# ShenhanQian/KGDet

Hardware: AMD Instinct MI355X
Metric: training images/sec (whole node) KGDet R50-FPN 800x1333 (higher is better)
Workload: dtype f32 (3 MFMA products per multiply on hi/lo-split operands -- fp16 parts forward, bf16 parts for gradients --, f32 accumulate); 1 GPU; KGDet R50-FPN train step, 2 img/GPU at 800x1333 (padded 800x1344), DeformConv fwd/bwd + focal/moment losses + grad-clip + Adam; no collective at dp1 (one rank: nothing to exchange); global_batch=2, parallelism=dp1

## Files before the change

### kgdet_amd/csrc/bn_act.hip

```cpp
#include "common.h"

namespace kgdet {

namespace {

__device__ __forceinline__ float wave_sum(float v) {
#pragma unroll
  for (int d = 32; d > 0; d >>= 1) v += __shfl_xor(v, d);
  return v;
}

struct ChannelAffine {
  float s, t, mean, invstd;
};

__device__ __forceinline__ ChannelAffine channel_affine(const float *gamma, const float *beta, const float *mean,
                                                        const float *var, float eps, int c) {
  ChannelAffine a;
  a.mean = mean[c];
  a.invstd = 1.0f / sqrtf(var[c] + eps);
  a.s = (gamma ? gamma[c] : 1.0f) * a.invstd;
  a.t = (beta ? beta[c] : 0.0f) - a.mean * a.s;
  return a;
}
// ... 95 lines not shown
__global__ __launch_bounds__(256) void relu_sum_bwd_kernel(const float *__restrict__ gz, const float *__restrict__ z,
                                                           float *__restrict__ g, float *__restrict__ partial, int C, int HW,
                                                           int per, int P) {
  __shared__ float red[4];
  const int plane = blockIdx.y, c = plane % C, n = plane / C;
  const long long base = (long long)plane * HW;
  const int lo = blockIdx.x * per, hi = min(HW, lo + per);
  float s1 = 0.f;
  {
    typedef float f32x4u __attribute__((ext_vector_type(4), aligned(4)));
    const int hi4 = lo + ((hi - lo) & ~3);
    for (int i = lo + threadIdx.x * 4; i < hi4; i += 1024) {
      f32x4u v = *reinterpret_cast<const f32x4u *>(gz + base + i);
      if (RELU) {
        const f32x4u zv = *reinterpret_cast<const f32x4u *>(z + base + i);
        v[0] = zv[0] > 0.f ? v[0] : 0.f; v[1] = zv[1] > 0.f ? v[1] : 0.f; v[2] = zv[2] > 0.f ? v[2] : 0.f; v[3] = zv[3] > 0.f ? v[3] : 0.f;
        *reinterpret_cast<f32x4u *>(g + base + i) = v;
      }
      s1 += (v[0] + v[1]) + (v[2] + v[3]);
    }
    for (int i = hi4 + threadIdx.x; i < hi; i += 256) {
      float v = gz[base + i];
      if (RELU) { v = z[base + i] > 0.f ? v : 0.f; g[base + i] = v; }
      s1 += v;
    }
  }
  s1 = wave_sum(s1);
  if ((threadIdx.x & 63) == 0) red[threadIdx.x >> 6] = s1;
  __syncthreads();
  if (threadIdx.x == 0) partial[(long long)c * P + n * gridDim.x + blockIdx.x] = (red[0] + red[1]) + (red[2] + red[3]);
}

__global__ __launch_bounds__(256) void bn_fold_finish_kernel(const float *__restrict__ partial, int P,
                                                             const float *__restrict__ w, float *__restrict__ G,
                                                             const float *__restrict__ s, const float *__restrict__ mean,
                                                             const float *__restrict__ var, float eps,
                                                             float *__restrict__ gbeta, float *__restrict__ ggamma, int CK) {
  __shared__ float red[2][4];
  const int o = blockIdx.x;
  float sb = 0.f;
  for (int k = threadIdx.x; k < P; k += 256) sb += partial[(long long)o * P + k];
  float dot = 0.f;
  const float so = s[o];
  const float *wr = w + (long long)o * CK;
  float *gr = G ? G + (long long)o * CK : nullptr;
  if (gr) {
    for (int k = threadIdx.x; k < CK; k += 256) {
      const float gv = gr[k];
      dot += wr[k] * gv;
      gr[k] = gv * so;
    }
  }
  sb = wave_sum(sb);
  dot = wave_sum(dot);
  if ((threadIdx.x & 63) == 0) { red[0][threadIdx.x >> 6] = sb; red[1][threadIdx.x >> 6] = dot; }
  __syncthreads();
  if (threadIdx.x == 0) {
    const float b = (red[0][0] + red[0][1]) + (red[0][2] + red[0][3]);
    const float d = (red[1][0] + red[1][1]) + (red[1][2] + red[1][3]);
    if (gbeta) gbeta[o] = b;
    if (ggamma) ggamma[o] = (d - mean[o] * b) / sqrtf(var[o] + eps);
  }
}

namespace {

int chunks_for(int64_t planes, int64_t HW) {
  int64_t want = (4096 + planes - 1) / planes;
  const int64_t most = (HW + 1023) / 1024;
  if (want > most) want = most;
  return want < 1 ? 1 : (int)want;
}

}

}

using namespace kgdet;

__global__ __launch_bounds__(256) void bn_relu_maxpool_kernel(const float *__restrict__ x, const float *__restrict__ gamma,
                                                              const float *__restrict__ beta,
                                                              const float *__restrict__ mean,
                                                              const float *__restrict__ var, float eps,
                                                              float *__restrict__ y, int C, int H, int W, int Ho, int Wo) {
  const int plane = blockIdx.y, c = plane % C;
  const ChannelAffine a = channel_affine(gamma, beta, mean, var, eps, c);
  const float *xp = x + (long long)plane * H * W;
  float *yp = y + (long long)plane * Ho * Wo;
  for (int o = blockIdx.x * 256 + threadIdx.x; o < Ho * Wo; o += gridDim.x * 256) {
    const int i = o / Wo, j = o - i * Wo;
    float m = 0.f;
#pragma unroll
    for (int dy = -1; dy <= 1; ++dy) {
      const int r = 2 * i + dy;
      if (r < 0 || r >= H) continue;
#pragma unroll
      for (int dx = -1; dx <= 1; ++dx) {
        const int q = 2 * j + dx;
        if (q < 0 || q >= W) continue;
        m = fmaxf(m, xp[(long long)r * W + q] * a.s + a.t);
      }
    }
    yp[o] = m;
  }
}

extern "C" int kgdet_bn_relu_maxpool(const float *x, const float *gamma, const float *beta, const float *mean,
                                     const float *var, float eps, float *y, int64_t N, int32_t C, int32_t H, int32_t W,
                                     void *stream) {
  KGDET_CHECK_SHAPE(N >= 0 && C > 0 && H > 0 && W > 0, "bad sizes");
  if (N == 0) return KGDET_OK;
  KGDET_CHECK_SHAPE(x && y && mean && var, "null pointer");
  KGDET_CHECK_SHAPE(N * C <= 65535, "N*C = %lld exceeds the grid limit", (long long)(N * C));
  const int Ho = (H - 1) / 2 + 1, Wo = (W - 1) / 2 + 1;
  int chunks = (Ho * Wo + 1023) / 1024;
  hipLaunchKernelGGL(bn_relu_maxpool_kernel, dim3(chunks, (unsigned)(N * C)), dim3(256), 0, (hipStream_t)stream, x, gamma,
                     beta, mean, var, eps, y, C, H, W, Ho, Wo);
  KGDET_CHECK_LAUNCH("bn_relu_maxpool");
  return KGDET_OK;
}

extern "C" int32_t kgdet_bn_act_partials(int64_t N, int32_t C, int64_t HW) {
  if (N <= 0 || C <= 0 || HW <= 0) return 0;
  return (int32_t)(N * chunks_for(N * C, HW));
}

extern "C" int kgdet_bn_act_forward(const float *x, const float *gamma, const float *beta, const float *mean,
                                    const float *var, float eps, const float *residual, float *y, int64_t N, int32_t C,
                                    int64_t HW, int32_t relu, void *stream) {
  KGDET_CHECK_SHAPE(N >= 0 && C > 0 && HW >= 0 && HW < (1LL << 31), "bad sizes");
  if (N * HW == 0) return KGDET_OK;
  KGDET_CHECK_SHAPE(x && y && mean && var, "null pointer");
  KGDET_CHECK_SHAPE(N * C <= 65535, "N*C = %lld exceeds the grid limit", (long long)(N * C));
  const int chunks = chunks_for(N * C, HW);
  const int per = (int)(((HW + chunks - 1) / chunks + 3) / 4 * 4);
  dim3 grid(chunks, (unsigned)(N * C));
#define LAUNCH(RES, RELU)                                                                                      \
  hipLaunchKernelGGL((bn_act_fwd_kernel<RES, RELU>), grid, dim3(256), 0, (hipStream_t)stream, x, gamma, beta, \
                     mean, var, eps, residual, y, C, (int)HW, per)
  if (residual) { if (relu) LAUNCH(true, true); else LAUNCH(true, false); }
  else { if (relu) LAUNCH(false, true); else LAUNCH(false, false); }
#undef LAUNCH
  KGDET_CHECK_LAUNCH("bn_act_forward");
  return KGDET_OK;
}

extern "C" int kgdet_bn_act_backward(const float *grad_y, const float *x, const float *y, const float *gamma,
                                     const float *beta, const float *mean, const float *var, float eps,
                                     int32_t has_residual, int32_t relu, float *grad_x, float *grad_residual,
                                     float *partial, float *sums, int64_t N, int32_t C, int64_t HW, void *stream) {
  KGDET_CHECK_SHAPE(N >= 0 && C > 0 && HW >= 0 && HW < (1LL << 31), "bad sizes");
  if (N * HW == 0) return KGDET_OK;
  KGDET_CHECK_SHAPE(grad_y && x && mean && var && partial, "null pointer");
  KGDET_CHECK_SHAPE(!(has_residual && relu) || (y && grad_residual),
                    "residual + relu needs the forward output and a grad_residual buffer");
  KGDET_CHECK_SHAPE(N * C <= 65535, "N*C = %lld exceeds the grid limit", (long long)(N * C));
  const int chunks = chunks_for(N * C, HW);
  const int per = (int)(((HW + chunks - 1) / chunks + 3) / 4 * 4);
  const int P = (int)(N * chunks);
  dim3 grid(chunks, (unsigned)(N * C));
#define LAUNCH(RES, RELU)                                                                                        \
  hipLaunchKernelGGL((bn_act_bwd_kernel<RES, RELU>), grid, dim3(256), 0, (hipStream_t)stream, grad_y, x, y, gamma, \
                     beta, mean, var, eps, grad_x, grad_residual, partial, C, (int)HW, per, P)
  if (has_residual) { if (relu) LAUNCH(true, true); else LAUNCH(true, false); }
  else { if (relu) LAUNCH(false, true); else LAUNCH(false, false); }
#undef LAUNCH
  KGDET_CHECK_LAUNCH("bn_act_backward");
  if (sums) {
    hipLaunchKernelGGL(bn_partial_sum, dim3((2 * C + 255) / 256), dim3(256), 0, (hipStream_t)stream, partial, sums, 2 * C,
                       P);
    KGDET_CHECK_LAUNCH("bn_partial_sum");
  }
  return KGDET_OK;
}

extern "C" int kgdet_bn_fold_backward(const float *grad_z, const float *z, int32_t relu, float *g, float *partial, int64_t N,
                                      int32_t C, int64_t HW, void *stream) {
  KGDET_CHECK_SHAPE(N >= 0 && C > 0 && HW >= 0 && HW < (1LL << 31), "bad sizes");
  if (N * HW == 0) return KGDET_OK;
  KGDET_CHECK_SHAPE(grad_z && partial && (!relu || (z && g)), "null pointer");
  KGDET_CHECK_SHAPE(N * C <= 65535, "N*C = %lld exceeds the grid limit", (long long)(N * C));
  const int chunks = chunks_for(N * C, HW);
  const int per = (int)(((HW + chunks - 1) / chunks + 3) / 4 * 4);
  const int P = (int)(N * chunks);
  dim3 grid(chunks, (unsigned)(N * C));
  if (relu)
    hipLaunchKernelGGL(relu_sum_bwd_kernel<true>, grid, dim3(256), 0, (hipStream_t)stream, grad_z, z, g, partial, C, (int)HW,
                       per, P);
  else
    hipLaunchKernelGGL(relu_sum_bwd_kernel<false>, grid, dim3(256), 0, (hipStream_t)stream, grad_z, z, g, partial, C,
                       (int)HW, per, P);
  KGDET_CHECK_LAUNCH("bn_fold_backward");
  return KGDET_OK;
}

extern "C" int kgdet_bn_fold_finish(const float *partial, int32_t P, const float *w, float *G, const float *s,
                                    const float *mean, const float *var, float eps, float *grad_beta, float *grad_gamma,
                                    int32_t O, int32_t CK, void *stream) {
  KGDET_CHECK_SHAPE(O > 0 && CK > 0 && P > 0, "bad sizes");
  KGDET_CHECK_SHAPE(partial && w && s && mean && var, "null pointer");
// ... 7 lines not shown
```

### kgdet_amd/csrc/dense_forward.hip

```cpp
#include "dense_common.h"

namespace kgdet {

__global__ __launch_bounds__(256) void conv1x1_pack(const float *__restrict__ w, int O, int C, int T, int transpose,
                                                    unsigned char *__restrict__ img, unsigned char *__restrict__ img_t,
                                                    int f16_forward) {
  if (gridDim.y == 2) {
    transpose = blockIdx.y;
    img = blockIdx.y ? img_t : img;
  }
  const bool f16 = f16_forward && !transpose;
  f16_saturate_on();
  const int M = transpose ? C : O, K = transpose ? O : C;
  const int k16s = (K + kTK - 1) / kTK;
  const long long total = (long long)((M + kTM - 1) / kTM) * k16s * T * 2 * kTM;
  for (long long i = blockIdx.x * 256LL + threadIdx.x; i < total; i += gridDim.x * 256LL) {
    const int row = (int)(i % kTM);
    const int khalf = (int)((i / kTM) & 1);
    const long long st = i / (2 * kTM);
    const int t = (int)(st % T);
    const int k16 = (int)((st / T) % k16s), mt = (int)(st / ((long long)T * k16s));
    const int m = mt * kTM + row, k0 = k16 * kTK + khalf * 8;
    float v[8];
#pragma unroll
    for (int j = 0; j < 8; ++j) {
      const long long o = transpose ? k0 + j : m, ch = transpose ? m : k0 + j;
      v[j] = (m < M && k0 + j < K) ? w[(o * C + ch) * T + (transpose ? T - 1 - t : t)] : 0.0f;
    }
    bf16x8 hi, lo;
    if (f16) {
#pragma unroll
      for (int j = 0; j < 8; ++j) v[j] *= kF16WeightScale;
      split8_t<true>(v, hi, lo);
    } else {
      split8(v, hi, lo);
    }
    unsigned char *dst = img + st * kStage + khalf * (kTM * 16) + row * 16;
    *reinterpret_cast<bf16x8 *>(dst) = hi;
    *reinterpret_cast<bf16x8 *>(dst + kPart) = lo;
  }
}

constexpr int kPackDescWords = 6;
__global__ __launch_bounds__(256) void conv1x1_pack_multi(const long long *__restrict__ desc, int n) {
  int lo = 0, hi = n - 1;
  while (lo < hi) {
    const int mid = (lo + hi + 1) >> 1;
    if ((int)(desc[mid * kPackDescWords + 4] & 0xffffffffLL) <= (int)blockIdx.x) lo = mid; else hi = mid - 1;
  }
  const long long *d = desc + lo * kPackDescWords;
  const float *w = reinterpret_cast<const float *>(d[0]);
  const float *scale = reinterpret_cast<const float *>(d[5]);
  const int O = (int)(d[3] >> 32), C = (int)(d[3] & 0xffffffffLL), T = (int)((d[4] >> 32) & 0xffff);
  const bool f16_forward = (d[4] >> 62) & 1;
  f16_saturate_on();
  const long long i = (long long)((int)blockIdx.x - (int)(d[4] & 0xffffffffLL)) * 256 + threadIdx.x;
#pragma unroll
  for (int transpose = 0; transpose < 2; ++transpose) {
    unsigned char *img = reinterpret_cast<unsigned char *>(d[1 + transpose]);
    const int M = transpose ? C : O, K = transpose ? O : C;
    const int k16s = (K + kTK - 1) / kTK;
    const long long total = (long long)((M + kTM - 1) / kTM) * k16s * T * 2 * kTM;
    if (!transpose && T == 9) {
      if (i >= total / 9) continue;
      const int row = (int)(i % kTM), khalf = (int)((i / kTM) & 1);
      const long long s2 = i / (2 * kTM);
      const int k16 = (int)(s2 % k16s), mt = (int)(s2 / k16s);
      const int m = mt * kTM + row, k0 = k16 * kTK + khalf * 8;
      float r[72];
      const f32x4 *src = reinterpret_cast<const f32x4 *>(w + ((long long)min(m, M - 1) * C + k0) * 9);
#pragma unroll
      for (int q = 0; q < 18; ++q) {
        const f32x4 u = src[q];
        r[4 * q] = u[0]; r[4 * q + 1] = u[1]; r[4 * q + 2] = u[2]; r[4 * q + 3] = u[3];
      }
      const float sc9 = (scale && m < M) ? scale[m] : 1.0f;
#pragma unroll
      for (int t = 0; t < 9; ++t) {
        float v[8];
#pragma unroll
        for (int j = 0; j < 8; ++j) v[j] = m < M ? r[j * 9 + t] * sc9 : 0.0f;
        bf16x8 hi8, lo8;
        if (f16_forward) {
#pragma unroll
          for (int j = 0; j < 8; ++j) v[j] *= kF16WeightScale;
          split8_t<true>(v, hi8, lo8);
        } else {
          split8(v, hi8, lo8);
        }
        unsigned char *dst = img + (s2 * 9 + t) * kStage + khalf * (kTM * 16) + row * 16;
        *reinterpret_cast<bf16x8 *>(dst) = hi8;
        *reinterpret_cast<bf16x8 *>(dst + kPart) = lo8;
      }
      continue;
    }
    if (i >= total) continue;
    const int row = (int)(i % kTM);
    const int khalf = (int)((i / kTM) & 1);
    const long long st = i / (2 * kTM);
    const int t = (int)(st % T);
    const int k16 = (int)((st / T) % k16s), mt = (int)(st / ((long long)T * k16s));
    const int m = mt * kTM + row, k0 = k16 * kTK + khalf * 8;
    float v[8];
#pragma unroll
    for (int j = 0; j < 8; ++j) {
      const long long o = transpose ? k0 + j : m, ch = transpose ? m : k0 + j;
      v[j] = (m < M && k0 + j < K) ? w[(o * C + ch) * T + (transpose ? T - 1 - t : t)] : 0.0f;
      if (scale && m < M && k0 + j < K) v[j] *= scale[o];
    }
    bf16x8 hi8, lo8;
    if (f16_forward && !transpose) {
#pragma unroll
      for (int j = 0; j < 8; ++j) v[j] *= kF16WeightScale;
      split8_t<true>(v, hi8, lo8);
    } else {
      split8(v, hi8, lo8);
    }
    unsigned char *dst = img + st * kStage + khalf * (kTM * 16) + row * 16;
    *reinterpret_cast<bf16x8 *>(dst) = hi8;
    *reinterpret_cast<bf16x8 *>(dst + kPart) = lo8;
  }
}

constexpr int kPF = 4;

template <int TAPS, int NW = 4, bool F16 = false>
__global__ __launch_bounds__(128 * NW) void conv_nn(const unsigned char *__restrict__ img,
                                                      const float *__restrict__ x, float *__restrict__ y, int M, int K,
                                                      int H, int W, int n_mt, int n_nt, int tiles, int ksplit,
                                                      long long part_stride, int Hin, int Win, int stride,
                                                      const float *__restrict__ bias,
                                                      const float *__restrict__ residual, int relu,
    const float *__restrict__ gate = nullptr) {
  constexpr int TN = 32 * NW, kPartB = 2 * TN * 16, kBuf = kStage + 2 * kPartB;
  __shared__ __attribute__((aligned(16))) unsigned char smem[2 * kBuf];
  if constexpr (F16) f16_saturate_on();
  const int unit = xcd_tile(blockIdx.x, tiles * ksplit);
  if (unit >= tiles * ksplit) return;
  const int part = unit % ksplit, tile = unit / ksplit;
  const int tid = threadIdx.x, lane = tid & 63, wave = tid >> 6, wm = wave & 1, wn = wave >> 1;
  const int n_local = tid % TN, kq = tid / TN;
  const int N = H * W;
  const int S = TAPS * ((K + kTK - 1) / kTK), per = (S + ksplit - 1) / ksplit;
  const int s_begin = part * per, s_end = max(s_begin, min(S, s_begin + per));
  const int stages = s_end - s_begin;
  struct Regs {
    f32x4 a;
    float v[4];
    unsigned live;
  };
  const int mt = tile % n_mt, nt = (tile / n_mt) % n_nt, b = tile / (n_mt * n_nt);
  const int n0 = nt * TN;
  const int p = min(n0 + n_local, N - 1);
  unsigned ok = 1u;
  if (TAPS == 9) {
    const int h = (p / W) * stride, w = (p - (p / W) * W) * stride;
    ok = 0u;
#pragma unroll
    for (int t = 0; t < 9; ++t) {
      const int hh = h + t / 3 - 1, ww = w + t % 3 - 1;
      ok |= (hh >= 0 && hh < Hin && ww >= 0 && ww < Win) ? (1u << t) : 0u;
    }
  }
  const int Nin = Hin * Win;
  const int pin = stride == 1 ? p : (p / W) * stride * Win + (p - (p / W) * W) * stride;
  const float *xb = x + (long long)b * K * Nin + pin;
  const unsigned char *ai = img + (long long)mt * S * kStage + (tid & 511) * 16;

  f32x16 acc[2];
#pragma unroll
  for (int i = 0; i < 2; ++i)
#pragma unroll
    for (int r = 0; r < 16; ++r) acc[i][r] = 0.0f;

  auto issue = [&](int s, Regs &R) {
    const int sc = s_begin + min(s, stages - 1);
    R.a = *reinterpret_cast<const f32x4 *>(ai + (long long)sc * kStage);
    const int c16 = sc / TAPS, t = sc - c16 * TAPS;
    int shift = 0;
    R.live = 1u;
    if (TAPS == 9) {
      R.live = (ok >> t) & 1u;
      shift = R.live ? (t / 3 - 1) * Win + (t % 3 - 1) : 0;
    }
    const float *xp = xb + (long long)(c16 * kTK + kq * 4) * Nin + shift;
    if (TAPS == 1 && (K & (kTK - 1)) && c16 == K / kTK) {
#pragma unroll
      for (int j = 0; j < 4; ++j) R.v[j] = xb[(long long)min(c16 * kTK + kq * 4 + j, K - 1) * Nin];
    } else {
#pragma unroll
      for (int j = 0; j < 4; ++j) R.v[j] = xp[(long long)j * Nin];
    }
  };
  auto commit = [&](int buf, const Regs &R) {
    unsigned char *As = smem + buf * kBuf, *Bs = As + kStage;
    *reinterpret_cast<f32x4 *>(As + (tid & 511) * 16) = R.a;
    uint2 hi, lo;
    split_pair_t<F16>(R.live ? R.v[0] : 0.0f, R.live ? R.v[1] : 0.0f, hi.x, lo.x);
    split_pair_t<F16>(R.live ? R.v[2] : 0.0f, R.live ? R.v[3] : 0.0f, hi.y, lo.y);
    unsigned char *dst = Bs + (kq >> 1) * (TN * 16) + n_local * 16 + (kq & 1) * 8;
    *reinterpret_cast<uint2 *>(dst) = hi;
    *reinterpret_cast<uint2 *>(dst + kPartB) = lo;
  };
  auto multiply = [&](int buf) {
// ... 529 lines not shown
    const long long u4 = (long long)n_mt * ((hw + 127) / 128) * B, u5 = (long long)n_mt * ((hw + 159) / 160) * B;
    const long long c4 = ((u4 + 255) / 256) * 4, c5 = ((u5 + 255) / 256) * 5;
    if (force_nw == 5 || (force_nw == 0 && u4 >= 200 && u5 >= 200 && c5 * 10 <= c4 * 9)) {
      p.NW = 5;
      p.n_nt = (int)((hw + 159) / 160);
    }
  }
  p.tiles = (long long)n_mt * p.n_nt * B;
  p.ks = nn_ksplit(p.tiles, taps * ((K + kTK - 1) / kTK));
  if (p.patch && p.tiles < 200) {
    const int chunks = K / kTK;
    double best = 1e30;
    p.ks = 1;
    for (int ks = 1; ks <= 8 && ks * 2 <= chunks; ++ks) {
      const double out_mb = (double)B * M * Ho * Wo * 4e-6;
      const double cost = (double)((p.tiles * ks + 255) / 256) * ((chunks + ks - 1) / ks) + 0.114 * out_mb * ks;
      if (cost < best) { best = cost; p.ks = ks; }
    }
  }
  static const int force_ks = env_int("KGDET_CONV_KS", 0);
  if (force_ks > 0) p.ks = force_ks;
  static const int force_halves = env_int("KGDET_CONV_HALVES", -1);
  p.halves = p.patch && p.NB == 4 &&
             (force_halves >= 0 ? force_halves != 0 : ((p.ks == 1 && p.tiles > 256 && p.tiles < 400) || M <= 64));
  return p;
}

enum NNCloser { kCloseStore = 0, kCloseSumEpilogue = 1, kCloseSumBiasAct = 2, kCloseSum = 3 };
NNCloser nn_closer(int ks, long long HW, bool epilogue) {
  if (ks <= 1) return kCloseStore;
  if (!epilogue) return kCloseSum;
  return HW % 2 == 0 ? kCloseSumEpilogue : kCloseSumBiasAct;
}

}

}

using namespace kgdet;

extern "C" size_t kgdet_conv_packed_bytes(int32_t M, int32_t K, int32_t taps) {
  if (M <= 0 || K <= 0 || (taps == 9 && K % kTK) || (taps != 1 && taps != 9)) return 0;
  return (size_t)pack_items(M, K, taps) * 32;
}

extern "C" int kgdet_conv_pack_fmt(const float *w, int32_t O, int32_t C, int32_t taps, int32_t transpose, void *packed,
                                   int32_t operand_format, void *stream) {
  const int M = transpose ? C : O, K = transpose ? O : C;
  KGDET_CHECK_SHAPE(taps == 1 || taps == 9, "taps must be 1 (1x1) or 9 (3x3)");
  KGDET_CHECK_SHAPE(O > 0 && C > 0 && (taps == 1 || K % kTK == 0), "reduction length %d is not a multiple of 16", K);
  KGDET_CHECK_SHAPE(w && packed, "null pointer");
  const long long blocks = (pack_items(M, K, taps) + 255) / 256;
  hipLaunchKernelGGL(conv1x1_pack, dim3((unsigned)(blocks > 65535 ? 65535 : blocks)), dim3(256), 0, (hipStream_t)stream, w,
                     O, C, taps, transpose, (unsigned char *)packed, (unsigned char *)nullptr, operand_format == 1 ? 1 : 0);
  KGDET_CHECK_LAUNCH("conv_pack");
  return KGDET_OK;
}

extern "C" int kgdet_conv_pack(const float *w, int32_t O, int32_t C, int32_t taps, int32_t transpose, void *packed,
                               void *stream) {
  return kgdet_conv_pack_fmt(w, O, C, taps, transpose, packed, 0, stream);
}

extern "C" int kgdet_conv_pack_both_fmt(const float *w, int32_t O, int32_t C, int32_t taps, void *packed, void *packed_t,
                                        int32_t forward_format, void *stream) {
  KGDET_CHECK_SHAPE(taps == 1 || taps == 9, "taps must be 1 (1x1) or 9 (3x3)");
  KGDET_CHECK_SHAPE(O > 0 && C > 0 && (taps == 1 || (O % kTK == 0 && C % kTK == 0)), "O and C must be multiples of 16");
  KGDET_CHECK_SHAPE(w && packed && packed_t, "null pointer");
  const long long blocks = pack_both_blocks(O, C, taps);
  hipLaunchKernelGGL(conv1x1_pack, dim3((unsigned)(blocks > 32768 ? 32768 : blocks), 2), dim3(256), 0,
                     (hipStream_t)stream, w, O, C, taps, 0, (unsigned char *)packed, (unsigned char *)packed_t,
                     forward_format == 1 ? 1 : 0);
  KGDET_CHECK_LAUNCH("conv_pack_both");
  return KGDET_OK;
}

extern "C" int kgdet_conv_pack_both(const float *w, int32_t O, int32_t C, int32_t taps, void *packed, void *packed_t,
                                    void *stream) {
  return kgdet_conv_pack_both_fmt(w, O, C, taps, packed, packed_t, 0, stream);
}

extern "C" int64_t kgdet_conv_pack_blocks(int32_t O, int32_t C, int32_t taps) {
  if (O <= 0 || C <= 0 || (taps == 9 && (O % kTK || C % kTK)) || (taps != 1 && taps != 9)) return 0;
  return pack_both_blocks(O, C, taps);
}

extern "C" int kgdet_conv_pack_multi(const int64_t *desc_dev, int32_t n, int64_t total_blocks, void *stream) {
  KGDET_CHECK_SHAPE(desc_dev && n > 0 && total_blocks > 0 && total_blocks < (1LL << 31), "bad descriptor table");
  hipLaunchKernelGGL(conv1x1_pack_multi, dim3((unsigned)total_blocks), dim3(256), 0, (hipStream_t)stream,
                     (const long long *)desc_dev, n);
  KGDET_CHECK_LAUNCH("conv_pack_multi");
  return KGDET_OK;
}

extern "C" size_t kgdet_conv_apply_workspace_bytes(int64_t B, int32_t M, int32_t K, int32_t H, int32_t W,
                                                    int32_t taps, int32_t stride) {
  if (B <= 0 || M <= 0 || K <= 0 || H <= 0 || W <= 0 || (taps == 9 && K % kTK) || stride < 1 || stride > 2) return 0;
  const long long HW = (long long)((H + stride - 1) / stride) * ((W + stride - 1) / stride);
  const int ks = plan_nn(B, M, K, H, W, taps, stride).ks;
  return ks > 1 ? (size_t)ks * B * M * HW * sizeof(float) : 0;
}

extern "C" int kgdet_conv_apply_plan(int64_t B, int32_t M, int32_t K, int32_t H, int32_t W, int32_t taps, int32_t stride,
                                     int32_t out[KGDET_CONV_APPLY_PLAN_WORDS]) {
  KGDET_CHECK_SHAPE(out, "null pointer");
  KGDET_CHECK_SHAPE(B > 0 && M > 0 && K > 0 && H > 0 && W > 0 && (long long)H * W < (1LL << 30), "bad sizes");
  KGDET_CHECK_SHAPE(taps == 1 || taps == 9, "taps must be 1 (1x1) or 9 (3x3)");
  KGDET_CHECK_SHAPE(stride == 1 || stride == 2, "stride must be 1 or 2");
  KGDET_CHECK_SHAPE(taps == 1 || K % kTK == 0, "reduction length %d is not a multiple of 16", K);
  const NNPlan p = plan_nn(B, M, K, H, W, taps, stride);
  KGDET_CHECK_SHAPE(p.tiles < (1LL << 28), "too many tiles");
  const long long HW = (long long)((H + stride - 1) / stride) * ((W + stride - 1) / stride);
  const int32_t words[KGDET_CONV_APPLY_PLAN_WORDS] = {
      p.patch, p.TX, p.TY, p.NB, p.NW, p.ks, p.halves, (int32_t)p.tiles, p.n_nt, nn_closer(p.ks, HW, true), nn_closer(p.ks, HW, false)};
  for (int i = 0; i < KGDET_CONV_APPLY_PLAN_WORDS; ++i) out[i] = words[i];
  return KGDET_OK;
}

extern "C" int kgdet_conv_apply_epilogue_fmt(const void *packed, const float *x, float *y, const float *bias,
                                             const float *residual, int32_t relu, int64_t B, int32_t M, int32_t K,
                                             int32_t H, int32_t W, int32_t taps, int32_t stride, int32_t operand_format,
                                             void *workspace, size_t workspace_bytes, void *stream) {
  return kgdet_conv_apply_gated_fmt(packed, x, y, bias, residual, relu, nullptr, B, M, K, H, W, taps, stride, operand_format,
                                    workspace, workspace_bytes, stream);
}

extern "C" int kgdet_conv_apply_gated_fmt(const void *packed, const float *x, float *y, const float *bias,
                                          const float *residual, int32_t relu, const float *gate, int64_t B, int32_t M,
                                          int32_t K, int32_t H, int32_t W, int32_t taps, int32_t stride,
                                          int32_t operand_format, void *workspace, size_t workspace_bytes, void *stream) {
  const bool f16 = operand_format == 1;
  KGDET_CHECK_SHAPE(B >= 0 && M > 0 && K > 0 && H >= 0 && W >= 0 && (long long)H * W < (1LL << 30), "bad sizes");
  KGDET_CHECK_SHAPE(taps == 1 || taps == 9, "taps must be 1 (1x1) or 9 (3x3)");
  KGDET_CHECK_SHAPE(stride == 1 || stride == 2, "stride must be 1 or 2");
  KGDET_CHECK_SHAPE(taps == 1 || K % kTK == 0, "reduction length %d is not a multiple of 16", K);
  const int Ho = (H + stride - 1) / stride, Wo = (W + stride - 1) / stride;
  const long long HW = (long long)Ho * Wo;
  if (B * HW == 0) return KGDET_OK;
  KGDET_CHECK_SHAPE(packed && x && y, "null pointer");
  const NNPlan plan = plan_nn(B, M, K, H, W, taps, stride);
  const int n_mt = (M + kTM - 1) / kTM, n_nt = plan.n_nt;
  const long long tiles = plan.tiles;
  KGDET_CHECK_SHAPE(tiles < (1LL << 28), "too many tiles");
  const int ks = plan.ks;
  const long long part_stride = B * M * HW;
  if (ks > 1) {
    KGDET_CHECK_SHAPE(workspace && workspace_bytes >= (size_t)ks * part_stride * sizeof(float), "workspace too small");
    KGDET_CHECK_SHAPE(part_stride % 2 == 0, "B*M*Ho*Wo must be even");
    KGDET_CHECK_SHAPE(!gate || HW % 2 == 0, "a gated K-split convolution needs an even pixel count");
  }
  const unsigned grid = (unsigned)((tiles * ks + 7) / 8) * 8;
  float *dst = ks > 1 ? (float *)workspace : y;
  const float *k_bias = ks > 1 ? nullptr : bias, *k_residual = ks > 1 ? nullptr : residual, *k_gate = ks > 1 ? nullptr : gate;
  const int k_relu = ks > 1 ? 0 : relu;
  const unsigned char *img = (const unsigned char *)packed;
  if (plan.patch) {
    auto launch = [&](auto bf16_kernel, auto f16_kernel, unsigned g, unsigned threads) {
      launch_fmt(f16, bf16_kernel, f16_kernel, g, threads, stream, img, x, dst, M, K, H, W, n_mt, plan.tiles_x, n_nt, (int)tiles,
                 ks, part_stride, plan.TX, plan.TY, k_bias, k_residual, k_relu, k_gate);
    };
    if (plan.NB == 5)
      launch(conv3x3_patch4<4, 5, false>, conv3x3_patch4<4, 5, true>, grid, 256);
    else if (plan.halves)
      launch(conv3x3_patch4<2, 4, false>, conv3x3_patch4<2, 4, true>, (unsigned)((tiles * ks * 2 + 7) / 8) * 8, 128);
    else
      launch(conv3x3_patch4<4, 4, false>, conv3x3_patch4<4, 4, true>, grid, 256);
  } else {
// ... 88 lines not shown
```

### kgdet_amd/csrc/dense_grad_weight.hip

```cpp
#include "dense_common.h"

namespace kgdet {

struct ConvFoldArgs {
  const float *w, *s, *mean, *var, *bn_partial;
  float *grad_beta, *grad_gamma;
  float eps;
  int P;
};
template <bool T9>
__global__ __launch_bounds__(1024) void conv_wsum_fold(const float *__restrict__ parts, float *__restrict__ out, int C,
                                                       long long stride, int count, const ConvFoldArgs f) {
  extern __shared__ float row_s[];
  __shared__ float red[2][16];
  const int o = blockIdx.x, CK = T9 ? 9 * C : C;
  const int nthr = blockDim.x, tid = threadIdx.x;
  const float so = f.s[o];
  const float *wr = f.w + (long long)o * CK;
  const float *pr = parts + (long long)o * CK;
  float *gr = out + (long long)o * CK;
  float dot = 0.0f, sb = 0.0f;
  for (int q = tid; q < CK; q += nthr) {
    float g0 = 0.0f;
    int k = 0;
// ... 394 lines not shown
#pragma unroll
        for (int pt = 0; pt < 2; ++pt) {
#pragma unroll
          for (int i = 0; i < 2; ++i) fa[ks][pt][i] = *reinterpret_cast<const bf16x8 *>(A + ks * kPKS + pt * kPPart + i * 32 * 16);
#pragma unroll
          for (int i = 0; i < kPNI; ++i) fb[ks][pt][i] = *reinterpret_cast<const bf16x8 *>(Bp + ks * kPKS + pt * kPPart + i * 32 * 16);
        }
#pragma unroll
      for (int ks = 0; ks < 2; ++ks) {
#pragma unroll
        for (int mi = 0; mi < 2; ++mi)
#pragma unroll
          for (int ni = 0; ni < kPNI; ++ni)
            acc[mi][ni] = __builtin_amdgcn_mfma_f32_32x32x16_bf16(fa[ks][1][mi], fb[ks][0][ni], acc[mi][ni], 0, 0, 0);
#pragma unroll
        for (int mi = 0; mi < 2; ++mi)
#pragma unroll
          for (int ni = 0; ni < kPNI; ++ni)
            acc[mi][ni] = __builtin_amdgcn_mfma_f32_32x32x16_bf16(fa[ks][0][mi], fb[ks][1][ni], acc[mi][ni], 0, 0, 0);
#pragma unroll
        for (int mi = 0; mi < 2; ++mi)
#pragma unroll
          for (int ni = 0; ni < kPNI; ++ni)
            acc[mi][ni] = __builtin_amdgcn_mfma_f32_32x32x16_bf16(fa[ks][0][mi], fb[ks][0][ni], acc[mi][ni], 0, 0, 0);
      }
    };
    if (n > 0) {
      __syncthreads();
      for (int j = 0; j < n; j += 2) {
        multiply(0);
        __syncthreads();
        if (j + 1 < n) {
          multiply(1);
          __syncthreads();
        }
      }
    }
    float *out = partial + (long long)split * M * N;
#pragma unroll
    for (int mi = 0; mi < 2; ++mi)
#pragma unroll
      for (int ni = 0; ni < kPNI; ++ni) {
        const int nn = nt * kTN + wn * (32 * kPNI) + ni * 32 + (lane & 31);
#pragma unroll
        for (int r = 0; r < 16; ++r) {
          const int m = mt * kTM + wm * 64 + mi * 32 + (r & 3) + 8 * (r >> 2) + 4 * (lane >> 5);
          if (m < M && nn < N) out[(long long)m * N + nn] = acc[mi][ni][r];
        }
      }
  }
}

template <int TAPS, bool ALIGNED>
__global__ __launch_bounds__(kPThreads, 1) void conv_ntp(const float *__restrict__ a, const float *__restrict__ bm,
                                                         float *__restrict__ partial, int M, int N, int L, int B, int n_mt,
                                                         int n_nt, int stages_per_image, int per, int H, int W, int Cin,
                                                         int units, float *__restrict__ row_sums = nullptr, int rs_stride = 0) {
  extern __shared__ __attribute__((aligned(16))) unsigned char smem[];
  const int unit = units > 0 ? xcd_tile(blockIdx.x, units) : (int)blockIdx.x;
  if (units > 0 && unit >= units) return;
  if (threadIdx.x >= kPCons * 64)
    conv_ntp_role<TAPS, true, ALIGNED>(a, bm, partial, M, N, L, B, n_mt, n_nt, stages_per_image, per, H, W, Cin, unit, smem, row_sums, rs_stride);
  else
    conv_ntp_role<TAPS, false, ALIGNED>(a, bm, partial, M, N, L, B, n_mt, n_nt, stages_per_image, per, H, W, Cin, unit, smem, row_sums, rs_stride);
}

}


__global__ __launch_bounds__(256) void pad_rows2(const float *__restrict__ a, float *__restrict__ ap, long long rows_a,
                                                 const float *__restrict__ b, float *__restrict__ bp, long long rows_b, int W,
                                                 int Wp) {
  const float *src = blockIdx.y ? b : a;
  float *dst = blockIdx.y ? bp : ap;
  const long long n = (blockIdx.y ? rows_b : rows_a) * Wp;
  for (long long i = (long long)blockIdx.x * 256 + threadIdx.x; i < n; i += (long long)gridDim.x * 256) {
    const long long r = i / Wp;
    const int c = (int)(i - r * Wp);
    dst[i] = c < W ? src[r * W + c] : 0.0f;
  }
}

__global__ __launch_bounds__(256) void conv_s2_gather9(const float *__restrict__ x, float *__restrict__ col, int C, int H, int W,
                                                       int Ho, int Wo, long long rows) {
  const int HWo = Ho * Wo;
  const long long total = rows * HWo;
  for (long long i = (long long)blockIdx.x * 256 + threadIdx.x; i < total; i += (long long)gridDim.x * 256) {
    const long long r = i / HWo;
    const int p = (int)(i - r * HWo), oy = p / Wo, ox = p - oy * Wo;
    const long long b = r / C;
    const int c = (int)(r - b * C);
    const float *xp = x + r * (long long)H * W;
    float *cp = col + (b * 9 * C + c) * (long long)HWo + p;
#pragma unroll
    for (int t = 0; t < 9; ++t) {
      const int yy = 2 * oy + t / 3 - 1, xx = 2 * ox + t % 3 - 1;
      cp[(long long)t * C * HWo] = (yy >= 0 && yy < H && xx >= 0 && xx < W) ? xp[(long long)yy * W + xx] : 0.0f;
    }
  }
}

namespace kgdet {

namespace {

int nt_splits(int tiles, int total_stages) {
  const int most = (total_stages + 31) / 32;
  double best = 1e30;
  const int s_max = 2 * ((256 + tiles - 1) / tiles) < 128 ? 2 * ((256 + tiles - 1) / tiles) : 128;
  for (int s = 1; s <= s_max; ++s) {
    const double t = (double)((tiles * s + 255) / 256) / s;
    if (t < best) best = t;
  }
  int splits = 0;
  for (int s = 1; s <= s_max && !splits; ++s)
    if ((double)((tiles * s + 255) / 256) / s <= best * (1.0 + 1e-9) && tiles * s >= 224 && tiles * s <= 256) splits = s;
  for (int s = s_max; s >= 1 && !splits; --s)
    if ((double)((tiles * s + 255) / 256) / s <= best * (1.0 + 1e-9)) splits = s;
  if (splits > most) splits = most;
  if (splits > 128) splits = 128;
  return splits < 1 ? 1 : splits;
}

int fold_threads(int cols) {
  const int t = (cols + 63) / 64 * 64;
  return t < 64 ? 64 : (t > 1024 ? 1024 : t);
}

struct GWPlan {
  int n_mt, n_nt, tiles, splits;
  bool use_ntp, padded;
  long long W, Wp, L, Lp;
  int spi, per;
  size_t copies_at, rows_at, bytes;
};
GWPlan plan_gw(long long B, int O, int C, long long H, long long W, int taps) {
  GWPlan p;
  p.W = W;
  p.Wp = (W + 3) & ~3LL;
  p.L = H * W;
  p.Lp = H * p.Wp;
  p.n_mt = (O + kTM - 1) / kTM;
  p.n_nt = taps == 9 ? 9 * C / kTN : (C + kTN - 1) / kTN;
  p.tiles = p.n_mt * p.n_nt;
  p.splits = nt_splits(p.tiles, (int)(B * ((p.Lp + kTK - 1) / kTK)));
  const long long widest = O > C ? O : C;
  p.use_ntp = taps == 9 ? W >= 4 && p.L >= 4 && p.L <= (1LL << 21) && widest * p.Lp < (1LL << 30)
                        : W % 4 != 0 && W >= 4 && widest * p.L < (1LL << 30);
  p.padded = W % 4 != 0 && !p.use_ntp;
  const long long stage = p.use_ntp ? kPK : kTK, len = p.use_ntp ? p.L : p.Lp;
  p.spi = (int)((len + stage - 1) / stage);
  p.per = (int)((B * p.spi + p.splits - 1) / p.splits);
  p.bytes = (size_t)p.splits * O * C * taps * sizeof(float);
  p.copies_at = align_up(p.bytes, 256);
  if (p.Wp != W) p.bytes = p.copies_at + (size_t)B * (O + C) * p.Lp * sizeof(float);
  p.rows_at = align_up(p.bytes, 256);
  p.bytes = p.rows_at + (size_t)p.splits * O * sizeof(float);
  return p;
}

int launch_gw(const GWPlan &p, int taps, const float *grad_y, const float *x, float *grad_w, long long B, int O, int C, int H,
              void *workspace, void *stream, const ConvFoldArgs *fold, int wsum_C) {
  unsigned char *ws = static_cast<unsigned char *>(workspace);
  const hipStream_t st = (hipStream_t)stream;
  float *partials = reinterpret_cast<float *>(ws);
  float *row_sums = (fold && !fold->bn_partial) ? reinterpret_cast<float *>(ws + p.rows_at) : nullptr;
  if (p.padded) {
    float *gyp = reinterpret_cast<float *>(ws + p.copies_at), *xp = gyp + (size_t)B * O * p.Lp;
// ... 79 lines not shown

}

using namespace kgdet;

extern "C" size_t kgdet_conv1x1_grad_weight_workspace_bytes(int64_t B, int32_t O, int32_t C, int64_t HW) {
  if (B <= 0 || O <= 0 || C <= 0 || HW <= 0) return 0;
  return plan_gw(B, O, C, 1, HW, 1).bytes;
}

extern "C" size_t kgdet_conv3x3_grad_weight_workspace_bytes(int64_t B, int32_t O, int32_t C, int32_t H, int32_t W) {
  if (B <= 0 || O <= 0 || C <= 0 || H <= 0 || W <= 0) return 0;
  return plan_gw(B, O, C, H, W, 9).bytes;
}

extern "C" int kgdet_conv_grad_weight_plan(int64_t B, int32_t O, int32_t C, int32_t H, int64_t W, int32_t taps,
                                           int32_t out[KGDET_CONV_GRAD_WEIGHT_PLAN_WORDS]) {
  KGDET_CHECK_SHAPE(out, "null pointer");
  KGDET_CHECK_SHAPE(taps == 1 || taps == 9, "taps must be 1 (1x1) or 9 (3x3)");
  if (taps == 9) {
    KGDET_CHECK_SHAPE(B > 0 && O > 0 && C > 0 && H > 0 && W > 0 && (long long)H * (W + 3) < (1LL << 23), "bad sizes");
    if (C % kTN != 0) {
      set_error("conv3x3_grad_weight needs C %% 128 == 0 (C=%d)", C);
      return KGDET_E_UNSUPPORTED;
    }
  } else {
    KGDET_CHECK_SHAPE(B > 0 && O > 0 && C > 0 && H == 1 && W > 0 && W < (1LL << 30), "bad sizes");
  }
  const GWPlan p = plan_gw(B, O, C, H, W, taps);
  KGDET_CHECK_SHAPE(p.bytes < ((size_t)1 << 39), "workspace beyond what the report can express");
  const int32_t words[KGDET_CONV_GRAD_WEIGHT_PLAN_WORDS] = {
      p.use_ntp, p.padded, p.W % 4 == 0, p.splits, p.spi, p.per, 0, (int32_t)(p.copies_at >> 8), (int32_t)(p.rows_at >> 8),
      p.tiles};
  for (int i = 0; i < KGDET_CONV_GRAD_WEIGHT_PLAN_WORDS; ++i) out[i] = words[i];
  return KGDET_OK;
}

extern "C" size_t kgdet_conv3x3_s2_grad_weight_workspace_bytes(int64_t B, int32_t O, int32_t C, int32_t H, int32_t W) {
  if (B <= 0 || O <= 0 || C <= 0 || H <= 0 || W <= 0) return 0;
  const long long HWo = (long long)((H + 1) / 2) * ((W + 1) / 2);
  return conv3x3_s2_col_bytes(B, C, H, W) + plan_gw(B, O, 9 * C, 1, HWo, 1).bytes;
}

extern "C" int kgdet_conv1x1_grad_weight(const float *grad_y, const float *x, float *grad_w, int64_t B, int32_t O,
                                         int32_t C, int64_t HW, void *workspace, size_t workspace_bytes,
                                         void *stream) {
  return grad_weight(1, grad_y, x, grad_w, B, O, C, 1, HW, workspace, workspace_bytes, stream, nullptr);
}

extern "C" int kgdet_conv1x1_grad_weight_fold(const float *grad_y, const float *x, float *grad_w, int64_t B, int32_t O,
                                              int32_t C, int64_t HW, void *workspace, size_t workspace_bytes, const float *w,
                                              const float *s, const float *mean, const float *var, float eps,
                                              const float *bn_partial, int32_t P, float *grad_beta, float *grad_gamma,
                                              void *stream) {
  ConvFoldArgs f;
  if (int rc = fold_args(f, w, s, mean, var, eps, bn_partial, P, grad_beta, grad_gamma)) return rc;
  return grad_weight(1, grad_y, x, grad_w, B, O, C, 1, HW, workspace, workspace_bytes, stream, &f);
}

extern "C" int kgdet_conv3x3_grad_weight(const float *grad_y, const float *x, float *grad_w, int64_t B, int32_t O,
                                         int32_t C, int32_t H, int32_t W, void *workspace, size_t workspace_bytes,
                                         void *stream) {
  return grad_weight(9, grad_y, x, grad_w, B, O, C, H, W, workspace, workspace_bytes, stream, nullptr);
}

extern "C" int kgdet_conv3x3_grad_weight_fold(const float *grad_y, const float *x, float *grad_w, int64_t B, int32_t O,
                                              int32_t C, int32_t H, int32_t W, void *workspace, size_t workspace_bytes,
                                              const float *w, const float *s, const float *mean, const float *var, float eps,
                                              const float *bn_partial, int32_t P, float *grad_beta, float *grad_gamma,
                                              void *stream) {
  ConvFoldArgs f;
  if (int rc = fold_args(f, w, s, mean, var, eps, bn_partial, P, grad_beta, grad_gamma)) return rc;
  return grad_weight(9, grad_y, x, grad_w, B, O, C, H, W, workspace, workspace_bytes, stream, &f);
}

extern "C" int kgdet_conv3x3_s2_grad_weight(const float *grad_y, const float *x, float *grad_w, int64_t B, int32_t O, int32_t C,
                                            int32_t H, int32_t W, void *workspace, size_t workspace_bytes, void *stream) {
  KGDET_CHECK_SHAPE(B > 0 && O > 0 && C > 0 && H > 0 && W > 0 && (long long)9 * C * ((H + 1) / 2) * ((W + 1) / 2) < (1LL << 30), "bad sizes");
  KGDET_CHECK_SHAPE(grad_y && x && grad_w && workspace, "null pointer");
  KGDET_CHECK_SHAPE(workspace_bytes >= kgdet_conv3x3_s2_grad_weight_workspace_bytes(B, O, C, H, W), "workspace too small");
  KGDET_CHECK_SHAPE(((long long)O * C) % 2 == 0, "O*C must be even");
  const int Ho = (H + 1) / 2, Wo = (W + 1) / 2;
  float *col = static_cast<float *>(workspace);
  const long long total = (long long)B * C * Ho * Wo;
  const long long blocks = (total + 255) / 256;
  hipLaunchKernelGGL(conv_s2_gather9, dim3((unsigned)(blocks > 16384 ? 16384 : blocks)), dim3(256), 0, (hipStream_t)stream, x, col, C,
                     H, W, Ho, Wo, (long long)B * C);
  KGDET_CHECK_LAUNCH("conv_s2_gather9");
  const size_t cb = conv3x3_s2_col_bytes(B, C, H, W);
  return grad_weight(1, grad_y, col, grad_w, B, O, 9 * C, 1, (long long)Ho * Wo, static_cast<unsigned char *>(workspace) + cb,
                     workspace_bytes - cb, stream, nullptr, C);
}
```

Baseline: 184.1 img/s.

## Vectorize maxpool and stride-2 gather; stage weight packing through shared-memory tiles

Adds vec4 paths to the fused BN-ReLU-maxpool kernel and to the stride-2 im2col gather. Each thread now produces four outputs from wide row loads and writes them with vector stores. Rewrites the multi-layer weight-pack kernel so each block loads a contiguous weight tile into shared memory and emits both the normal and transposed hi/lo images from it, replacing strided global reads. This aims to cut uncoalesced global traffic in small memory-bound kernels, at the cost of more complex indexing, shared-memory use and alignment-dependent dispatch.

Result: slower. 147.8 img/s (-19.7%).

```diff
diff --git a/kgdet_amd/csrc/bn_act.hip b/kgdet_amd/csrc/bn_act.hip
--- a/kgdet_amd/csrc/bn_act.hip
+++ b/kgdet_amd/csrc/bn_act.hip
@@ -201,11 +201,58 @@
                                                               const float *__restrict__ beta,
                                                               const float *__restrict__ mean,
                                                               const float *__restrict__ var, float eps,
-                                                              float *__restrict__ y, int C, int H, int W, int Ho, int Wo) {
+                                                              float *__restrict__ y, int C, int H, int W, int Ho, int Wo,
+                                                              int vec4) {
   const int plane = blockIdx.y, c = plane % C;
   const ChannelAffine a = channel_affine(gamma, beta, mean, var, eps, c);
   const float *xp = x + (long long)plane * H * W;
   float *yp = y + (long long)plane * Ho * Wo;
+  if (vec4) {
+    typedef float f32x4 __attribute__((ext_vector_type(4)));
+    typedef float f32x2 __attribute__((ext_vector_type(2)));
+    const int Wq = (Wo + 3) >> 2;
+    const bool wide = (Wo & 3) == 0;
+    for (int o = blockIdx.x * 256 + threadIdx.x; o < Ho * Wq; o += gridDim.x * 256) {
+      const int i = o / Wq, j0 = (o - i * Wq) * 4;
+      const bool full = j0 + 4 <= Wo;
+      float v[3][9];
+      bool have[3];
+#pragma unroll
+      for (int dy = 0; dy < 3; ++dy) {
+        const int r = 2 * i + dy - 1;
+        have[dy] = r >= 0;
+        const float *row = xp + (long long)(have[dy] ? r : 0) * W + 2 * j0;
+        const f32x4 zero = {0.f, 0.f, 0.f, 0.f};
+        const f32x4 p = *reinterpret_cast<const f32x4 *>(row), q = full ? *reinterpret_cast<const f32x4 *>(row + 4) : zero;
+        const float e = j0 > 0 ? row[-1] : 0.0f;
+        v[dy][0] = e * a.s + a.t;
+        v[dy][1] = p[0] * a.s + a.t; v[dy][2] = p[1] * a.s + a.t; v[dy][3] = p[2] * a.s + a.t; v[dy][4] = p[3] * a.s + a.t;
+        v[dy][5] = q[0] * a.s + a.t; v[dy][6] = q[1] * a.s + a.t; v[dy][7] = q[2] * a.s + a.t; v[dy][8] = q[3] * a.s + a.t;
+      }
+      f32x4 m = {0.f, 0.f, 0.f, 0.f};
+#pragma unroll
+      for (int k = 0; k < 4; ++k) {
+#pragma unroll
+        for (int dy = 0; dy < 3; ++dy) {
+          if (!have[dy]) continue;
+#pragma unroll
+          for (int dx = 0; dx < 3; ++dx) {
+            if (k == 0 && dx == 0 && j0 == 0) continue;
+            m[k] = fmaxf(m[k], v[dy][2 * k + dx]);
+          }
+        }
+      }
+      float *dst = yp + (long long)i * Wo + j0;
+      if (wide) {
+        *reinterpret_cast<f32x4 *>(dst) = m;
+      } else {
+        const f32x2 m0 = {m[0], m[1]}, m1 = {m[2], m[3]};
+        *reinterpret_cast<f32x2 *>(dst) = m0;
+        if (full) *reinterpret_cast<f32x2 *>(dst + 2) = m1;
+      }
+    }
+    return;
+  }
   for (int o = blockIdx.x * 256 + threadIdx.x; o < Ho * Wo; o += gridDim.x * 256) {
     const int i = o / Wo, j = o - i * Wo;
     float m = 0.f;
@@ -232,9 +279,10 @@
   KGDET_CHECK_SHAPE(x && y && mean && var, "null pointer");
   KGDET_CHECK_SHAPE(N * C <= 65535, "N*C = %lld exceeds the grid limit", (long long)(N * C));
   const int Ho = (H - 1) / 2 + 1, Wo = (W - 1) / 2 + 1;
+  const int vec4 = H % 2 == 0 && W % 4 == 0 && ((uintptr_t)x | (uintptr_t)y) % 16 == 0;
   int chunks = (Ho * Wo + 1023) / 1024;
   hipLaunchKernelGGL(bn_relu_maxpool_kernel, dim3(chunks, (unsigned)(N * C)), dim3(256), 0, (hipStream_t)stream, x, gamma,
-                     beta, mean, var, eps, y, C, H, W, Ho, Wo);
+                     beta, mean, var, eps, y, C, H, W, Ho, Wo, vec4);
   KGDET_CHECK_LAUNCH("bn_relu_maxpool");
   return KGDET_OK;
 }
diff --git a/kgdet_amd/csrc/dense_forward.hip b/kgdet_amd/csrc/dense_forward.hip
--- a/kgdet_amd/csrc/dense_forward.hip
+++ b/kgdet_amd/csrc/dense_forward.hip
@@ -42,7 +42,104 @@
 }
 
 constexpr int kPackDescWords = 6;
+constexpr int kPackTileFloats = 32 * (16 * 9 + 1);
+constexpr int pack_rows(int T) { return T == 9 ? 32 : 128; }
+static long long pack_multi_blocks(int O, int C, int T) {
+  return (long long)((O + kTM - 1) / kTM) * (kTM / pack_rows(T)) * ((C + kTM - 1) / kTM) * (kTM / kTK);
+}
+
+template <int T>
+__device__ __forceinline__ void pack_cell(const float *__restrict__ w, unsigned char *__restrict__ img,
+                                          unsigned char *__restrict__ img_t, const float *__restrict__ scale, int O, int C,
+                                          bool f16_forward, int cell, float *tile) {
+  constexpr int ROWS = pack_rows(T), RUN = kTK * T, LD = RUN + 1;
+  constexpr int PIECES = RUN / 4 + 1;
+  constexpr int TSTEP = 256 / (2 * ROWS);
+  const int tid = threadIdx.x;
+  const int n_cc = ((C + kTM - 1) / kTM) * (kTM / kTK);
+  const int rg = cell / n_cc, cc = cell - rg * n_cc;
+  const int o_base = rg * ROWS, c_base = cc * kTK;
+  const int k16s = (C + kTK - 1) / kTK, k16s_t = (O + kTK - 1) / kTK;
+  const int cols = c_base < C ? min(kTK, C - c_base) * T : 0;
+  for (int idx = tid; idx < ROWS * PIECES; idx += 256 * 4) {
+    float v[4][4];
+    int e0[4], row[4];
+#pragma unroll
+    for (int u = 0; u < 4; ++u) {
+      const int id = idx + 256 * u;
+      row[u] = id / PIECES;
+      const int piece = id - row[u] * PIECES, o = o_base + row[u];
+      const int L = (id < ROWS * PIECES && o < O) ? cols : 0;
+      const float *run = w + ((long long)min(o, O - 1) * C + min(c_base, C - 1)) * T;
+      const int a = (int)((reinterpret_cast<uintptr_t>(run) >> 2) & 3);
+      e0[u] = 4 * piece - a;
+      if (e0[u] >= 0 && e0[u] + 4 <= L) {
+        const f32x4 q = *reinterpret_cast<const f32x4 *>(run + e0[u]);
+        v[u][0] = q[0]; v[u][1] = q[1]; v[u][2] = q[2]; v[u][3] = q[3];
+      } else {
+#pragma unroll
+        for (int i = 0; i < 4; ++i) v[u][i] = (e0[u] + i >= 0 && e0[u] + i < L) ? run[e0[u] + i] : 0.0f;
+      }
+      if (scale && L > 0) {
+        const float sc = scale[o];
+#pragma unroll
+        for (int i = 0; i < 4; ++i)
+          if (e0[u] + i >= 0 && e0[u] + i < L) v[u][i] *= sc;
+      }
+    }
+#pragma unroll
+    for (int u = 0; u < 4; ++u) {
+      if (idx + 256 * u >= ROWS * PIECES) continue;
+#pragma unroll
+      for (int i = 0; i < 4; ++i)
+        if (e0[u] + i >= 0 && e0[u] + i < RUN) tile[row[u] * LD + e0[u] + i] = v[u][i];
+    }
+  }
+  __syncthreads();
+  if (cc < k16s) {
+    const int row = tid & (ROWS - 1), khalf = (tid / ROWS) & 1;
+    const int mt = o_base / kTM, row_in = (o_base & (kTM - 1)) + row;
+    unsigned char *dst0 = img + (long long)(mt * k16s + cc) * T * kStage + khalf * (kTM * 16) + row_in * 16;
+    const float *src = tile + row * LD + khalf * 8 * T;
+    for (int t = tid / (2 * ROWS); t < T; t += TSTEP) {
+      float v[8];
+#pragma unroll
+      for (int j = 0; j < 8; ++j) v[j] = src[j * T + t];
+      bf16x8 hi8, lo8;
+      if (f16_forward) {
+#pragma unroll
+        for (int j = 0; j < 8; ++j) v[j] *= kF16WeightScale;
+        split8_t<true>(v, hi8, lo8);
+      } else {
+        split8(v, hi8, lo8);
+      }
+      unsigned char *dst = dst0 + (long long)t * kStage;
+      *reinterpret_cast<bf16x8 *>(dst) = hi8;
+      *reinterpret_cast<bf16x8 *>(dst + kPart) = lo8;
+    }
+  }
+  {
+    const int c = tid & 15, khalf = (tid >> 4) & 1, og = (tid >> 5) & (ROWS / kTK - 1);
+    const int mt_t = cc >> 3, row_t = (cc & 7) * kTK + c, k16 = o_base / kTK + og;
+    if (k16 < k16s_t) {
+      unsigned char *dst0 = img_t + (long long)(mt_t * k16s_t + k16) * T * kStage + khalf * (kTM * 16) + row_t * 16;
+      const float *src = tile + (og * kTK + khalf * 8) * LD + c * T + (T - 1);
+      for (int t = tid / (2 * ROWS); t < T; t += TSTEP) {
+        float v[8];
+#pragma unroll
+        for (int j = 0; j < 8; ++j) v[j] = src[j * LD - t];
+        bf16x8 hi8, lo8;
+        split8(v, hi8, lo8);
+        unsigned char *dst = dst0 + (long long)t * kStage;
+        *reinterpret_cast<bf16x8 *>(dst) = hi8;
+        *reinterpret_cast<bf16x8 *>(dst + kPart) = lo8;
+      }
+    }
+  }
+}
+
 __global__ __launch_bounds__(256) void conv1x1_pack_multi(const long long *__restrict__ desc, int n) {
+  __shared__ float tile[kPackTileFloats];
   int lo = 0, hi = n - 1;
   while (lo < hi) {
     const int mid = (lo + hi + 1) >> 1;
@@ -54,72 +151,10 @@
   const int O = (int)(d[3] >> 32), C = (int)(d[3] & 0xffffffffLL), T = (int)((d[4] >> 32) & 0xffff);
   const bool f16_forward = (d[4] >> 62) & 1;
   f16_saturate_on();
-  const long long i = (long long)((int)blockIdx.x - (int)(d[4] & 0xffffffffLL)) * 256 + threadIdx.x;
-#pragma unroll
-  for (int transpose = 0; transpose < 2; ++transpose) {
-    unsigned char *img = reinterpret_cast<unsigned char *>(d[1 + transpose]);
-    const int M = transpose ? C : O, K = transpose ? O : C;
-    const int k16s = (K + kTK - 1) / kTK;
-    const long long total = (long long)((M + kTM - 1) / kTM) * k16s * T * 2 * kTM;
-    if (!transpose && T == 9) {
-      if (i >= total / 9) continue;
-      const int row = (int)(i % kTM), khalf = (int)((i / kTM) & 1);
-      const long long s2 = i / (2 * kTM);
-      const int k16 = (int)(s2 % k16s), mt = (int)(s2 / k16s);
-      const int m = mt * kTM + row, k0 = k16 * kTK + khalf * 8;
-      float r[72];
-      const f32x4 *src = reinterpret_cast<const f32x4 *>(w + ((long long)min(m, M - 1) * C + k0) * 9);
-#pragma unroll
-      for (int q = 0; q < 18; ++q) {
-        const f32x4 u = src[q];
-        r[4 * q] = u[0]; r[4 * q + 1] = u[1]; r[4 * q + 2] = u[2]; r[4 * q + 3] = u[3];
-      }
-      const float sc9 = (scale && m < M) ? scale[m] : 1.0f;
-#pragma unroll
-      for (int t = 0; t < 9; ++t) {
-        float v[8];
-#pragma unroll
-        for (int j = 0; j < 8; ++j) v[j] = m < M ? r[j * 9 + t] * sc9 : 0.0f;
-        bf16x8 hi8, lo8;
-        if (f16_forward) {
-#pragma unroll
-          for (int j = 0; j < 8; ++j) v[j] *= kF16WeightScale;
-          split8_t<true>(v, hi8, lo8);
-        } else {
-          split8(v, hi8, lo8);
-        }
-        unsigned char *dst = img + (s2 * 9 + t) * kStage + khalf * (kTM * 16) + row * 16;
-        *reinterpret_cast<bf16x8 *>(dst) = hi8;
-        *reinterpret_cast<bf16x8 *>(dst + kPart) = lo8;
-      }
-      continue;
-    }
-    if (i >= total) continue;
-    const int row = (int)(i % kTM);
-    const int khalf = (int)((i / kTM) & 1);
-    const long long st = i / (2 * kTM);
-    const int t = (int)(st % T);
-    const int k16 = (int)((st / T) % k16s), mt = (int)(st / ((long long)T * k16s));
-    const int m = mt * kTM + row, k0 = k16 * kTK + khalf * 8;
-    float v[8];
-#pragma unroll
-    for (int j = 0; j < 8; ++j) {
-      const long long o = transpose ? k0 + j : m, ch = transpose ? m : k0 + j;
-      v[j] = (m < M && k0 + j < K) ? w[(o * C + ch) * T + (transpose ? T - 1 - t : t)] : 0.0f;
-      if (scale && m < M && k0 + j < K) v[j] *= scale[o];
-    }
-    bf16x8 hi8, lo8;
-    if (f16_forward && !transpose) {
-#pragma unroll
-      for (int j = 0; j < 8; ++j) v[j] *= kF16WeightScale;
-      split8_t<true>(v, hi8, lo8);
-    } else {
-      split8(v, hi8, lo8);
-    }
-    unsigned char *dst = img + st * kStage + khalf * (kTM * 16) + row * 16;
-    *reinterpret_cast<bf16x8 *>(dst) = hi8;
-    *reinterpret_cast<bf16x8 *>(dst + kPart) = lo8;
-  }
+  const int cell = (int)blockIdx.x - (int)(d[4] & 0xffffffffLL);
+  unsigned char *img = reinterpret_cast<unsigned char *>(d[1]), *img_t = reinterpret_cast<unsigned char *>(d[2]);
+  if (T == 9) pack_cell<9>(w, img, img_t, scale, O, C, f16_forward, cell, tile);
+  else pack_cell<1>(w, img, img_t, scale, O, C, f16_forward, cell, tile);
 }
 
 constexpr int kPF = 4;
@@ -815,7 +850,7 @@
 
 extern "C" int64_t kgdet_conv_pack_blocks(int32_t O, int32_t C, int32_t taps) {
   if (O <= 0 || C <= 0 || (taps == 9 && (O % kTK || C % kTK)) || (taps != 1 && taps != 9)) return 0;
-  return pack_both_blocks(O, C, taps);
+  return pack_multi_blocks(O, C, taps);
 }
 
 extern "C" int kgdet_conv_pack_multi(const int64_t *desc_dev, int32_t n, int64_t total_blocks, void *stream) {
diff --git a/kgdet_amd/csrc/dense_grad_weight.hip b/kgdet_amd/csrc/dense_grad_weight.hip
--- a/kgdet_amd/csrc/dense_grad_weight.hip
+++ b/kgdet_amd/csrc/dense_grad_weight.hip
@@ -500,8 +500,54 @@
 }
 
 __global__ __launch_bounds__(256) void conv_s2_gather9(const float *__restrict__ x, float *__restrict__ col, int C, int H, int W,
-                                                       int Ho, int Wo, long long rows) {
+                                                       int Ho, int Wo, long long rows, int vec4) {
   const int HWo = Ho * Wo;
+  if (vec4) {
+    using kgdet::f32x2;
+    using kgdet::f32x4;
+    const int Wq = (Wo + 3) >> 2, HWq = Ho * Wq;
+    const bool wide = (Wo & 3) == 0;
+    const long long total = rows * HWq;
+    for (long long i = (long long)blockIdx.x * 256 + threadIdx.x; i < total; i += (long long)gridDim.x * 256) {
+      const long long r = i / HWq;
+      const int q = (int)(i - r * HWq), oy = q / Wq, ox0 = (q - oy * Wq) * 4;
+      const bool full = ox0 + 4 <= Wo;
+      const long long b = r / C;
+      const int c = (int)(r - b * C);
+      const float *xp = x + r * (long long)H * W + 2 * ox0;
+      float v[3][9];
+#pragma unroll
+      for (int ky = 0; ky < 3; ++ky) {
+        const int yy = 2 * oy + ky - 1;
+        if (yy >= 0) {
+          const float *row = xp + (long long)yy * W;
+          const f32x4 zero = {0.0f, 0.0f, 0.0f, 0.0f};
+          const f32x4 a = *reinterpret_cast<const f32x4 *>(row), d = full ? *reinterpret_cast<const f32x4 *>(row + 4) : zero;
+          v[ky][0] = ox0 > 0 ? row[-1] : 0.0f;
+          v[ky][1] = a[0]; v[ky][2] = a[1]; v[ky][3] = a[2]; v[ky][4] = a[3];
+          v[ky][5] = d[0]; v[ky][6] = d[1]; v[ky][7] = d[2]; v[ky][8] = d[3];
+        } else {
+#pragma unroll
+          for (int k = 0; k < 9; ++k) v[ky][k] = 0.0f;
+        }
+      }
+      float *cp = col + (b * 9 * C + c) * (long long)HWo + oy * Wo + ox0;
+#pragma unroll
+      for (int t = 0; t < 9; ++t) {
+        const int ky = t / 3, kx = t % 3;
+        float *dst = cp + (long long)t * C * HWo;
+        if (wide) {
+          const f32x4 o = {v[ky][kx], v[ky][kx + 2], v[ky][kx + 4], v[ky][kx + 6]};
+          *reinterpret_cast<f32x4 *>(dst) = o;
+        } else {
+          const f32x2 o0 = {v[ky][kx], v[ky][kx + 2]}, o1 = {v[ky][kx + 4], v[ky][kx + 6]};
+          *reinterpret_cast<f32x2 *>(dst) = o0;
+          if (full) *reinterpret_cast<f32x2 *>(dst + 2) = o1;
+        }
+      }
+    }
+    return;
+  }
   const long long total = rows * HWo;
   for (long long i = (long long)blockIdx.x * 256 + threadIdx.x; i < total; i += (long long)gridDim.x * 256) {
     const long long r = i / HWo;
@@ -747,10 +793,11 @@
   KGDET_CHECK_SHAPE(((long long)O * C) % 2 == 0, "O*C must be even");
   const int Ho = (H + 1) / 2, Wo = (W + 1) / 2;
   float *col = static_cast<float *>(workspace);
-  const long long total = (long long)B * C * Ho * Wo;
+  const int vec4 = H % 2 == 0 && W % 4 == 0 && ((uintptr_t)x | (uintptr_t)col) % 16 == 0;
+  const long long total = vec4 ? (long long)B * C * Ho * ((Wo + 3) / 4) : (long long)B * C * Ho * Wo;
   const long long blocks = (total + 255) / 256;
   hipLaunchKernelGGL(conv_s2_gather9, dim3((unsigned)(blocks > 16384 ? 16384 : blocks)), dim3(256), 0, (hipStream_t)stream, x, col, C,
-                     H, W, Ho, Wo, (long long)B * C);
+                     H, W, Ho, Wo, (long long)B * C, vec4);
   KGDET_CHECK_LAUNCH("conv_s2_gather9");
   const size_t cb = conv3x3_s2_col_bytes(B, C, H, W);
   return grad_weight(1, grad_y, col, grad_w, B, O, 9 * C, 1, (long long)Ho * Wo, static_cast<unsigned char *>(workspace) + cb,
```
